# TaoMiner/joint-kg-recommender

Measured on NVIDIA H100. Metric: scored (h,r,t) triples/s, TransE d=100 forward + margin loss + backward, higher is better.
Workload: dtype f32

## Files before the change

joint-kg-recommender_b200/csrc/train_group.cu:

```cuda
#include <cstdlib>
#include "train_dev.cuh"

namespace kgrec {

struct GroupArgs {
  kgrec_tables T;
  const void *ph, *pt, *pr;
  int is64;
  const int32_t* corrupt;
  LossCfg L;
  float keep;
};

__device__ __forceinline__ const float* row_ptr(const float* base, uint32_t row, uint32_t ld) {
  return base + static_cast<uint64_t>(row) * ld;
}

template <int FAM, int NCH>
struct GroupPos {
  using R = Row<NCH, true>;
  static constexpr int NE = R::NE;
  float h[NE], t[NE], w[NE];
  float base_h[NE];
  float base_t[NE];
// ... 496 lines not shown
      goff += d4;
    };

    for (int k = 0; k < K; k += 2) {
      if (k + 1 < K) {
        idb = ent_id(__shfl_sync(FULL, cv, k + 1), headb);
        if (act) xb = ldg_f4_hint(row(ent_b, idb), pol_keep);
      }
      negative(xa, heada, ida, k);
      if (k + 1 < K) {
        if (k + 2 < K) {
          ida = ent_id(__shfl_sync(FULL, cv, k + 2), heada);
          if (act) xa = ldg_f4_hint(row(ent_b, ida), pol_keep);
        }
        negative(xb, headb, idb, k + 1);
      }
    }
    const float cp = cpos * up;
    const float4 eps = make_float4(cp * ddist_term(ep.x, L1), cp * ddist_term(ep.y, L1), cp * ddist_term(ep.z, L1), cp * ddist_term(ep.w, L1));
    float4 gh = make_float4(accT.x + eps.x, accT.y + eps.y, accT.z + eps.z, accT.w + eps.w);
    float4 gt = make_float4(accH.x - eps.x, accH.y - eps.y, accH.z - eps.z, accH.w - eps.w);
    float4 gr = make_float4(accT.x - accH.x + eps.x, accT.y - accH.y + eps.y, accT.z - accH.z + eps.z, accT.w - accH.w + eps.w);
    if (REG) {
      const float mh = 1.f + n_tail, mt = 1.f + (static_cast<float>(K) - n_tail), mr = 1.f + static_cast<float>(K);
      lreg += mh * fmaxf(nh2 - 1.f, 0.f) + mt * fmaxf(nt2 - 1.f, 0.f) + mr * fmaxf(nr2 - 1.f, 0.f);
      const float ch = nh2 > 1.f ? mh * r2 : 0.f, ct = nt2 > 1.f ? mt * r2 : 0.f, cr = nr2 > 1.f ? mr * r2 : 0.f;
      gh.x = fmaf(ch, h.x, gh.x); gh.y = fmaf(ch, h.y, gh.y); gh.z = fmaf(ch, h.z, gh.z); gh.w = fmaf(ch, h.w, gh.w);
      gt.x = fmaf(ct, t.x, gt.x); gt.y = fmaf(ct, t.y, gt.y); gt.z = fmaf(ct, t.z, gt.z); gt.w = fmaf(ct, t.w, gt.w);
      gr.x = fmaf(cr, r.x, gr.x); gr.y = fmaf(cr, r.y, gr.y); gr.z = fmaf(cr, r.z, gr.z); gr.w = fmaf(cr, r.w, gr.w);
    }
    if (!BWD) {
      if (lane == 0) {
        pos_scores[j] = sp;
        group_loss[j] = lsum + (REG ? lreg : 0.f);
      }
      if (lane < K) neg_scores[static_cast<uint32_t>(j) * K + lane] = mys;
    }
    if (!FWD && act) {
      if (DENSE) {
        red_add_f4(reinterpret_cast<float*>(gent_b + static_cast<uint64_t>(ih0) * d4), gh.x, gh.y, gh.z, gh.w);
        red_add_f4(reinterpret_cast<float*>(gent_b + static_cast<uint64_t>(it0) * d4), gt.x, gt.y, gt.z, gt.w);
        red_add_f4(reinterpret_cast<float*>(grel_b + static_cast<uint64_t>(ir0) * d4), gr.x, gr.y, gr.z, gr.w);
      } else {
        const uint32_t g0 = static_cast<uint32_t>(j) * (2 + K) * d4;
        stg_f4_hint(reinterpret_cast<float4*>(gent_b + g0), gh.x, gh.y, gh.z, gh.w, pol_stream);
        stg_f4_hint(reinterpret_cast<float4*>(gent_b + g0 + d4), gt.x, gt.y, gt.z, gt.w, pol_stream);
        stg_f4_hint(reinterpret_cast<float4*>(grel_b + static_cast<uint32_t>(j) * d4), gr.x, gr.y, gr.z, gr.w, pol_stream);
      }
    }
  }
  if (bad && status) *status = 1;
}

template <bool L1, bool DENSE, bool MARGIN, int W>
__global__ void __launch_bounds__(W * 32, 1)
k_group_step_e_tma(const GroupArgs G, const float up0, float* __restrict__ pos_scores, float* __restrict__ neg_scores,
                   float* __restrict__ group_loss, const kgrec_grads Gr, int64_t* __restrict__ slot_ent,
                   int64_t* __restrict__ slot_rel, int32_t* status, const int S) {
  extern __shared__ __align__(128) unsigned char smem_raw[];
  const kgrec_tables& T = G.T;
  const LossCfg& L = G.L;
  const int lane = threadIdx.x & 31, wid = threadIdx.x >> 5;
  const int K = L.n_neg, n_rows = 3 + K;
  const int n_pos = static_cast<int>(L.n_pos);
  const uint32_t n_ent = static_cast<uint32_t>(T.n_ent);
  const uint32_t ld4 = static_cast<uint32_t>(T.ld) * 4u, d4 = static_cast<uint32_t>(T.dim) * 4u;
  const int bp = static_cast<int>(L.batch_pos < 0x7fffffff ? L.batch_pos : 0x7fffffff);
  const uint64_t pol_stream = policy_evict_first();
  const bool act = lane * 4 < T.dim;
  uint64_t* bars = reinterpret_cast<uint64_t*>(smem_raw) + wid * S;
  int32_t* ids_ring = reinterpret_cast<int32_t*>(smem_raw + static_cast<size_t>(W) * S * 8) + wid * S * 32;
  const uint32_t stage_bytes = static_cast<uint32_t>(n_rows) * d4;
  unsigned char* rows_base = smem_raw + ((static_cast<size_t>(W) * S * (8 + 128) + 127) & ~static_cast<size_t>(127)) +
                             static_cast<size_t>(wid) * S * stage_bytes;
  if (lane == 0)
    for (int s = 0; s < S; ++s) mbar_init(bars + s, 1);
  mbar_fence_init();
  __syncwarp();
  char* gent_b = reinterpret_cast<char*>(Gr.ent) + lane * 16;
  char* grel_b = reinterpret_cast<char*>(Gr.rel) + lane * 16;
  const float prm = L.param;
  const int stride = gridDim.x * W;
  const float4 z4 = make_float4(0.f, 0.f, 0.f, 0.f);
  bool bad = false;
  const void* pcol = lane == 0 ? G.ph : (lane == 1 ? G.pt : G.pr);

  auto issue = [&](int jj, int s) {
    int32_t v = 0;
    if (lane < 3) {
      const int64_t pv = load_idx(pcol, jj, G.is64);
      const int64_t lim = lane == 2 ? T.n_rel : T.n_ent;
      if (static_cast<uint64_t>(pv) >= static_cast<uint64_t>(lim)) bad = true; else v = static_cast<int32_t>(pv);
    } else if (lane < n_rows) {
      v = __ldg(G.corrupt + static_cast<uint32_t>(jj) * K + (lane - 3));
      const uint32_t id = static_cast<uint32_t>(v < 0 ? ~v : v);
      if (id >= n_ent) { bad = true; v = 0; }
    }
    ids_ring[s * 32 + lane] = v;
    if (lane == 0) mbar_arrive_expect_tx(bars + s, stage_bytes);
    __syncwarp();
    if (lane < n_rows) {
      const uint32_t id = lane < 3 ? static_cast<uint32_t>(v) : static_cast<uint32_t>(v < 0 ? ~v : v);
      const char* src = reinterpret_cast<const char*>(lane == 2 ? T.rel : T.ent) + static_cast<uint64_t>(id) * ld4;
      bulk_g2s(rows_base + static_cast<size_t>(s) * stage_bytes + static_cast<size_t>(lane) * d4, src, d4, bars + s);
    }
  };

  int j = blockIdx.x * W + wid;
  for (int s = 0, jj = j; s < S - 1 && jj < n_pos; ++s, jj += stride) issue(jj, s);
  for (int it = 0; j < n_pos; j += stride, ++it) {
    const int s = it % S;
    {
      const int jn = j + (S - 1) * stride;
      if (jn < n_pos) {
        fence_proxy_async_smem();
        __syncwarp();
        issue(jn, (it + S - 1) % S);
      }
    }
    mbar_wait(bars + s, static_cast<uint32_t>(it / S) & 1u);
    const int32_t myid = ids_ring[s * 32 + lane];
    const uint32_t st_addr = smem_u32(rows_base + static_cast<size_t>(s) * stage_bytes) + lane * 16;
    const uint32_t ih0 = static_cast<uint32_t>(__shfl_sync(FULL, myid, 0)), it0 = static_cast<uint32_t>(__shfl_sync(FULL, myid, 1)),
                   ir0 = static_cast<uint32_t>(__shfl_sync(FULL, myid, 2));
    if (slot_ent) {
      const uint32_t s0 = static_cast<uint32_t>(j) * (2 + K);
      if (lane < 2) slot_ent[s0 + lane] = myid;
      if (lane == 2) slot_rel[j] = myid;
      if (lane >= 3 && lane < n_rows) slot_ent[s0 + lane - 1] = myid < 0 ? ~myid : myid;
    }
    float4 h = z4, t = z4, r = z4;
    if (act) { h = lds_f4(st_addr); t = lds_f4(st_addr + d4); r = lds_f4(st_addr + 2 * d4); }
    float up = up0;
    if (!MARGIN) {
      const int b = j / bp;
      up /= static_cast<float>(min(bp, n_pos - b * bp)) * static_cast<float>(K);
    }
    const float4 bh = make_float4(h.x + r.x, h.y + r.y, h.z + r.z, h.w + r.w);
    const float4 bt = make_float4(t.x - r.x, t.y - r.y, t.z - r.z, t.w - r.w);
    const float4 ep = make_float4(bh.x - t.x, bh.y - t.y, bh.z - t.z, bh.w - t.w);
    const float sp = warp_sum(dist_term(ep.x, L1) + dist_term(ep.y, L1) + dist_term(ep.z, L1) + dist_term(ep.w, L1));
    float lsum = 0.f, cpos = 0.f, mys = 0.f;
    float4 accT = z4, accH = z4;
    uint32_t goff = (static_cast<uint32_t>(j) * (2 + K) + 2) * d4;
#pragma unroll 2
    for (int k = 0; k < K; ++k) {
      const int32_t c = __shfl_sync(FULL, myid, 3 + k);
      const bool head = c < 0;
      const uint32_t id = static_cast<uint32_t>(head ? ~c : c);
      float4 x = z4;
      if (act) x = lds_f4(st_addr + (3 + k) * d4);
      const float4 B = head ? bt : bh;
      const float4 e = make_float4(B.x - x.x, B.y - x.y, B.z - x.z, B.w - x.w);
      const float sn = warp_sum(dist_term(e.x, L1) + dist_term(e.y, L1) + dist_term(e.z, L1) + dist_term(e.w, L1));
      if (lane == k) mys = sn;
      float coef;
      if (MARGIN) {
        const float tt = sp - sn + prm;
        lsum += fmaxf(tt, 0.f);
        coef = tt > 0.f ? up : 0.f;
        cpos += tt > 0.f ? 1.f : 0.f;
      } else {
        const float xx = prm * (sp - sn);
        lsum += fmaxf(-xx, 0.f) + log1pf(expf(-fabsf(xx)));
        const float dp = -prm / (1.f + expf(xx));
        cpos += dp;
        coef = dp * up;
      }
      if (coef != 0.f) {
        float4 gc;
        if (L1) {
          gc = make_float4(coef * ddist_term(e.x, 1), coef * ddist_term(e.y, 1), coef * ddist_term(e.z, 1), coef * ddist_term(e.w, 1));
        } else {
          const float c2 = 2.f * coef;
          gc = make_float4(c2 * e.x, c2 * e.y, c2 * e.z, c2 * e.w);
        }
        if (head) { accH.x -= gc.x; accH.y -= gc.y; accH.z -= gc.z; accH.w -= gc.w; }
        else { accT.x -= gc.x; accT.y -= gc.y; accT.z -= gc.z; accT.w -= gc.w; }
        if (act) {
          if (DENSE) red_add_f4(reinterpret_cast<float*>(gent_b + static_cast<uint64_t>(id) * d4), gc.x, gc.y, gc.z, gc.w);
          else stg_f4_hint(reinterpret_cast<float4*>(gent_b + goff), gc.x, gc.y, gc.z, gc.w, pol_stream);
        }
      } else if (!DENSE) {
        if (act) stg_f4_hint(reinterpret_cast<float4*>(gent_b + goff), 0.f, 0.f, 0.f, 0.f, pol_stream);
      }
      goff += d4;
    }
    const float cp = cpos * up;
    const float4 eps = make_float4(cp * ddist_term(ep.x, L1), cp * ddist_term(ep.y, L1), cp * ddist_term(ep.z, L1), cp * ddist_term(ep.w, L1));
    const float4 gh = make_float4(accT.x + eps.x, accT.y + eps.y, accT.z + eps.z, accT.w + eps.w);
    const float4 gt = make_float4(accH.x - eps.x, accH.y - eps.y, accH.z - eps.z, accH.w - eps.w);
    const float4 gr = make_float4(accT.x - accH.x + eps.x, accT.y - accH.y + eps.y, accT.z - accH.z + eps.z, accT.w - accH.w + eps.w);
    if (lane == 0) {
      pos_scores[j] = sp;
      group_loss[j] = lsum;
    }
    if (lane < K) neg_scores[static_cast<uint32_t>(j) * K + lane] = mys;
    if (act) {
      if (DENSE) {
        red_add_f4(reinterpret_cast<float*>(gent_b + static_cast<uint64_t>(ih0) * d4), gh.x, gh.y, gh.z, gh.w);
        red_add_f4(reinterpret_cast<float*>(gent_b + static_cast<uint64_t>(it0) * d4), gt.x, gt.y, gt.z, gt.w);
        red_add_f4(reinterpret_cast<float*>(grel_b + static_cast<uint64_t>(ir0) * d4), gr.x, gr.y, gr.z, gr.w);
      } else {
        const uint32_t g0 = static_cast<uint32_t>(j) * (2 + K) * d4;
        stg_f4_hint(reinterpret_cast<float4*>(gent_b + g0), gh.x, gh.y, gh.z, gh.w, pol_stream);
        stg_f4_hint(reinterpret_cast<float4*>(gent_b + g0 + d4), gt.x, gt.y, gt.z, gt.w, pol_stream);
        stg_f4_hint(reinterpret_cast<float4*>(grel_b + static_cast<uint32_t>(j) * d4), gr.x, gr.y, gr.z, gr.w, pol_stream);
      }
    }
  }
  if (bad && status) *status = 1;
}

template <bool L1, bool DENSE, bool MARGIN, int MINB, bool PF, bool REG, bool BWD, bool FWD = false>
__global__ void __launch_bounds__(kThreads, MINB)
k_group_step_h(const GroupArgs G, const float up0, const float* __restrict__ up_dev, float* __restrict__ pos_scores,
               float* __restrict__ neg_scores, float* __restrict__ group_loss, const kgrec_grads Gr,
               int64_t* __restrict__ slot_ent, int64_t* __restrict__ slot_rel, int32_t* status) {
  const kgrec_tables& T = G.T;
  const LossCfg& L = G.L;
  const int lane = threadIdx.x & 31, wid = threadIdx.x >> 5;
  const int K = L.n_neg;
  const int n_pos = static_cast<int>(L.n_pos);
  const uint32_t n_ent = static_cast<uint32_t>(T.n_ent);
  const uint32_t ld4 = static_cast<uint32_t>(T.ld) * 4u, d4 = static_cast<uint32_t>(T.dim) * 4u;
  const int bp = static_cast<int>(L.batch_pos < 0x7fffffff ? L.batch_pos : 0x7fffffff);
  const uint64_t pol_keep = policy_evict_last(G.keep), pol_stream = policy_evict_first();
  const bool act = lane * 4 < T.dim;
  const char* ent_b = reinterpret_cast<const char*>(T.ent) + lane * 16;
  const char* rel_b = reinterpret_cast<const char*>(T.rel) + lane * 16;
  const char* nrm_b = reinterpret_cast<const char*>(T.norm) + lane * 16;
  char* gent_b = reinterpret_cast<char*>(Gr.ent) + lane * 16;
  char* grel_b = reinterpret_cast<char*>(Gr.rel) + lane * 16;
  char* gnrm_b = reinterpret_cast<char*>(Gr.norm) + lane * 16;
  const float prm = L.param;
  const int stride = gridDim.x * kWarpsPerCta;
  const float4 z4 = make_float4(0.f, 0.f, 0.f, 0.f);
  auto row = [&](const char* base, uint32_t id) { return reinterpret_cast<const float4*>(base + static_cast<uint64_t>(id) * ld4); };
  auto dot4 = [](const float4& a, const float4& b) { return fmaf(a.x, b.x, fmaf(a.y, b.y, fmaf(a.z, b.z, a.w * b.w))); };
  bool bad = false;
  auto ent_id = [&](int32_t c, bool& head) {
    head = c < 0;
    uint32_t id = static_cast<uint32_t>(head ? ~c : c);
    if (id >= n_ent) { bad = true; id = 0; }
    return id;
  };
  int j = blockIdx.x * kWarpsPerCta + wid;
  const void* pcol = lane == 0 ? G.ph : (lane == 1 ? G.pt : G.pr);
  auto fetch_ids = [&](int jj, int32_t& cv, int64_t& pv) {
    cv = lane < K ? __ldg(G.corrupt + static_cast<uint32_t>(jj) * K + lane) : 0;
    pv = lane < 3 ? load_idx(pcol, jj, G.is64) : 0;
  };
  int32_t cv = 0, cvn = 0;
  int64_t pv = 0, pvn = 0;
  if (j < n_pos) fetch_ids(j, cvn, pvn);
  for (; j < n_pos; j += stride) {
    cv = cvn;
    pv = pvn;
    const int jn = j + stride;
    if (jn < n_pos) fetch_ids(jn, cvn, pvn);
    const int64_t vh = __shfl_sync(FULL, pv, 0), vt = __shfl_sync(FULL, pv, 1), vr = __shfl_sync(FULL, pv, 2);
    uint32_t ih = static_cast<uint32_t>(vh), it = static_cast<uint32_t>(vt), ir = static_cast<uint32_t>(vr);
    if (static_cast<uint64_t>(vh) >= static_cast<uint64_t>(T.n_ent)) { bad = true; ih = 0; }
    if (static_cast<uint64_t>(vt) >= static_cast<uint64_t>(T.n_ent)) { bad = true; it = 0; }
    if (static_cast<uint64_t>(vr) >= static_cast<uint64_t>(T.n_rel)) { bad = true; ir = 0; }
    if (slot_ent) {
      const uint32_t s0 = static_cast<uint32_t>(j) * (2 + K);
      if (lane < 2) slot_ent[s0 + lane] = pv;
      if (lane == 2) slot_rel[j] = pv;
      if (lane < K) slot_ent[s0 + 2 + lane] = cv < 0 ? ~cv : cv;
    }
    float4 h = z4, t = z4, r = z4, w = z4, xa = z4, xb = z4;
    bool heada, headb = false;
    uint32_t ida = ent_id(__shfl_sync(FULL, cv, 0), heada), idb = 0;
    if (act) {
      h = ldg_f4_hint(row(ent_b, ih), pol_keep);
      t = ldg_f4_hint(row(ent_b, it), pol_keep);
      r = ldg_f4_hint(row(rel_b, ir), pol_keep);
      w = ldg_f4_hint(row(nrm_b, ir), pol_keep);
      xa = ldg_f4_hint(row(ent_b, ida), pol_keep);
    }
    if (PF && lane >= 2 && lane < K) {
      const uint32_t pid = static_cast<uint32_t>(cv < 0 ? ~cv : cv);
      if (pid < n_ent) {
        const char* pr = reinterpret_cast<const char*>(T.ent) + static_cast<uint64_t>(pid) * ld4;
        for (uint32_t o = 0; o < d4; o += 128) prefetch_l1(pr + o);
      }
    }
    float up = up0;
    if (BWD && up_dev) up *= __ldg(up_dev + j / bp);
    if (!MARGIN) {
      const int b = j / bp;
      up /= static_cast<float>(min(bp, n_pos - b * bp)) * static_cast<float>(K);
    }
    [[maybe_unused]] const float svec = (BWD && lane < K) ? __ldg(neg_scores + static_cast<uint32_t>(j) * K + lane) : 0.f;
    float a = dot4(h, w), b = dot4(t, w);
    warp_sum2(a, b);
    const float4 pt = make_float4(fmaf(-b, w.x, t.x), fmaf(-b, w.y, t.y), fmaf(-b, w.z, t.z), fmaf(-b, w.w, t.w));
    const float4 bh = make_float4(fmaf(-a, w.x, h.x) + r.x, fmaf(-a, w.y, h.y) + r.y, fmaf(-a, w.z, h.z) + r.z, fmaf(-a, w.w, h.w) + r.w);
    const float4 bt = make_float4(pt.x - r.x, pt.y - r.y, pt.z - r.z, pt.w - r.w);
    const float4 ep = make_float4(bh.x - pt.x, bh.y - pt.y, bh.z - pt.z, bh.w - pt.w);
    const float sp = BWD ? __ldg(pos_scores + j)
                         : warp_sum(dist_term(ep.x, L1) + dist_term(ep.y, L1) + dist_term(ep.z, L1) + dist_term(ep.w, L1));
    float lsum = 0.f, cpos = 0.f, mys = 0.f, sT = 0.f, sH = 0.f;
    float4 accT = z4, accH = z4, gwv = z4;
    uint32_t goff = (static_cast<uint32_t>(j) * (2 + K) + 2) * d4;
    [[maybe_unused]] float nh2 = 0.f, nt2 = 0.f, nr2 = 0.f, wr = 0.f, lreg = 0.f, n_tail = 0.f;
// ... 581 lines not shown
        if (MARGIN) {
          const float tt = sp - sn + prm;
          lsum += fmaxf(tt, 0.f);
          coef = tt > 0.f ? -up : 0.f;
          cpos += tt > 0.f ? 1.f : 0.f;
        } else {
          const float xx = prm * (sp - sn);
          lsum += fmaxf(-xx, 0.f) + log1pf(expf(-fabsf(xx)));
          const float dp = -prm / (1.f + expf(xx));
          cpos += dp;
          coef = -dp * up;
        }
#pragma unroll
        for (int i = 0; i < 4; ++i) {
          const int a = lane + 32 * i;
          const float g = coef * ddist_term(e[i], l1);
          gp[i] += g;
          if (head) gt[i] -= g; else gh[i] += g;
          if (a < d) Yc[a] = head ? g : -g;
        }
      }
      const float cp = cpos * up;
#pragma unroll
      for (int i = 0; i < 4; ++i) {
        const int a = lane + 32 * i;
        const float g = cp * ddist_term(yh[i] + rr[i] - yt[i], l1);
        gp[i] += g;
        if (a < d) {
          Y[a] = gh[i] + g;
          Y[pitch + a] = gt[i] - g;
          if (Gr.mode == 0) Gr.rel[static_cast<int64_t>(j) * d + a] = gp[i];
          else atomicAdd(Gr.rel + static_cast<uint64_t>(rel) * d + a, gp[i]);
        }
      }
      if (lane == 0) { pos_scores[j] = sp; group_loss[j] = lsum; }
      if (lane < K) neg_scores[static_cast<int64_t>(j) * K + lane] = mys;
    }
    if (wid == kWarpsPerCta - 1) plan(buf ^ 1, i0 + ng);
    __syncthreads();
    if (mt) {
      const float4* gp[QA];
      const ulonglong2* vp[QB];
#pragma unroll
      for (int qa = 0; qa < QA; ++qa) gp[qa] = reinterpret_cast<const float4*>(sG + 4 * min(ta + nta * qa, NC - 1));
#pragma unroll
      for (int q = 0; q < QB; ++q) vp[q] = reinterpret_cast<const ulonglong2*>(sV + 4 * min(tb + ntb * q, NC - 1));
      const int p4 = pitch >> 2;
#pragma unroll 2
      for (int n = 0; n < rows; ++n) {
        float4 g[QA];
        ulonglong2 v[QB];
#pragma unroll
        for (int qa = 0; qa < QA; ++qa) { g[qa] = *gp[qa]; gp[qa] += p4; }
#pragma unroll
        for (int q = 0; q < QB; ++q) { v[q] = *vp[q]; vp[q] += p4; }
#pragma unroll
        for (int qa = 0; qa < QA; ++qa) {
          const float gs[4] = {g[qa].x, g[qa].y, g[qa].z, g[qa].w};
#pragma unroll
          for (int r = 0; r < 4; ++r) {
            const f32x2 s2 = splat2(gs[r]);
#pragma unroll
            for (int q = 0; q < QB; ++q) {
              accM[4 * qa + r][q][0] = fma2(s2, v[q].x, accM[4 * qa + r][q][0]);
              accM[4 * qa + r][q][1] = fma2(s2, v[q].y, accM[4 * qa + r][q][1]);
            }
          }
        }
      }
    }
    __syncthreads();
    copy_rows();
#pragma unroll 1
    for (int rb = 0; rb < RB; ++rb) {
      const int base = 8 * (wid + kWarpsPerCta * rb);
      if (base >= rows) break;
      const int dense = Gr.mode;
      float* const* dstp = sDst + buf * ROWS + base;
      run_tile_dot<QF>(sG + base * pitch, sMt, d, NC, pitch, lane, [&](int i, int b, float v) {
        if (base + i < rows) {
          float* dst = dstp[i] + b;
          if (dense) atomicAdd(dst, v); else __stcs(dst, v);
        }
      });
    }
    asm volatile("cp.async.wait_group 0;" ::: "memory");
    __syncthreads();
    i0 += ng;
    buf ^= 1;
  }
  flush(cur_rel);
  if (bad && status) *status = 1;
}

__global__ void __launch_bounds__(256)
k_group_slot_ids(const void* ph, const void* pt, const void* pr, const int is64, const int32_t* __restrict__ corrupt,
                 const int64_t n_pos, const int K, int64_t* __restrict__ slot_ent, int64_t* __restrict__ slot_rel) {
  const int64_t total = n_pos * (2 + K);
  for (int64_t i = static_cast<int64_t>(blockIdx.x) * blockDim.x + threadIdx.x; i < total; i += static_cast<int64_t>(gridDim.x) * blockDim.x) {
    const int64_t j = i / (2 + K);
    const int t = static_cast<int>(i - j * (2 + K));
    int64_t v;
    if (t == 0) { v = load_idx(ph, j, is64); slot_rel[j] = load_idx(pr, j, is64); }
    else if (t == 1) v = load_idx(pt, j, is64);
    else { const int32_t c = __ldg(corrupt + j * K + (t - 2)); v = c < 0 ? ~c : c; }
    slot_ent[i] = v;
  }
}

__global__ void __launch_bounds__(256)
k_rel_hist(const void* pr, const int is64, const int n_pos, const int64_t n_rel, int32_t* __restrict__ count) {
  for (int j = blockIdx.x * blockDim.x + threadIdx.x; j < n_pos; j += gridDim.x * blockDim.x) {
    int64_t r = load_idx(pr, j, is64);
    if (static_cast<uint64_t>(r) >= static_cast<uint64_t>(n_rel)) r = 0;
    atomicAdd(count + r, 1);
  }
}

__global__ void __launch_bounds__(1024)
k_rel_scan(int32_t* __restrict__ count, const int64_t n_rel) {
  __shared__ int32_t part[1024];
  const int64_t per = (n_rel + 1023) / 1024, lo = threadIdx.x * per, hi = lo + per < n_rel ? lo + per : n_rel;
  int32_t s = 0;
  for (int64_t r = lo; r < hi; ++r) s += count[r];
  part[threadIdx.x] = s;
  __syncthreads();
  for (int off = 1; off < 1024; off <<= 1) {
    const int32_t v = threadIdx.x >= off ? part[threadIdx.x - off] : 0;
    __syncthreads();
    part[threadIdx.x] += v;
    __syncthreads();
  }
  int32_t run = part[threadIdx.x] - s;
  for (int64_t r = lo; r < hi; ++r) { const int32_t c = count[r]; count[r] = run; run += c; }
}

__global__ void __launch_bounds__(256)
k_rel_scatter(const void* pr, const int is64, const int n_pos, const int64_t n_rel, int32_t* __restrict__ cursor,
              int32_t* __restrict__ order) {
  for (int j = blockIdx.x * blockDim.x + threadIdx.x; j < n_pos; j += gridDim.x * blockDim.x) {
    int64_t r = load_idx(pr, j, is64);
    if (static_cast<uint64_t>(r) >= static_cast<uint64_t>(n_rel)) r = 0;
    order[atomicAdd(cursor + r, 1)] = j;
  }
}

int make_plan(const kgrec_tables* T, int model, Plan* pl);

static const char* group_step_env() {
  static const char* cached = [] { const char* e = getenv("KGREC_GROUP_STEP"); return e ? e : ""; }();
  return cached[0] ? cached : nullptr;
}

static int group_step_tma_mode(const kgrec_tables* T, int n_neg, int reg_flags) {
  const char* env = group_step_env();
  if (reg_flags) return 0;
  if (env && env[0] == 't' && env[1] && env[2]) {
    const int W = env[1] == '8' ? 8 : (env[1] == 'c' ? 12 : 16), S = env[2] - '0';
    if (S < 2 || S > 6) return 0;
    const size_t smem = static_cast<size_t>(W) * S * (136 + static_cast<size_t>(3 + n_neg) * T->dim * 4) + 128;
    return smem <= 225 * 1024 ? 16 * W + S : 0;
  }
  return 0;
}

static int group_check(const kgrec_tables* T, int model, Plan* pl, const void* ph, const void* pt, const void* pr,
                       int idx_bytes, int64_t n_pos, const int32_t* corrupt, int32_t n_neg, int64_t batch_pos,
                       int loss_kind, bool allow_r = false) {
  int rc = make_plan(T, model, pl);
  if (rc) return rc;
  if (pl->fam != FAM_E && pl->fam != FAM_H && !(allow_r && pl->fam == FAM_R)) {
    set_error("corrupt-format ranking loss is built for TransE / TransH (model %d)", model);
    return KGREC_ERR_UNSUPPORTED;
  }
  if (!pl->vec) { set_error("corrupt-format ranking loss needs embedding_size %% 4 == 0 and 16-byte aligned tables"); return KGREC_ERR_UNSUPPORTED; }
  if (idx_bytes != 4 && idx_bytes != 8) { set_error("idx_bytes must be 4 or 8"); return KGREC_ERR_INVALID; }
  if (!ph || !pt || !pr || !corrupt) { set_error("index array is NULL"); return KGREC_ERR_INVALID; }
  if (loss_kind != KGREC_LOSS_MARGIN && loss_kind != KGREC_LOSS_BPR) { set_error("unknown loss %d", loss_kind); return KGREC_ERR_INVALID; }
  if (n_pos < 0 || n_pos > 0x7fffffff || n_neg < 1 || batch_pos < 1) { set_error("bad n_pos / n_neg / batch_pos"); return KGREC_ERR_INVALID; }
  if (T->n_ent > 0x7fffffffll) { set_error("corrupt format holds entity ids in 31 bits"); return KGREC_ERR_UNSUPPORTED; }
  return KGREC_OK;
}

}

using namespace kgrec;

#define KGREC_GROUP_DISPATCH(CALL)                                            \
  if (pl.fam == FAM_E) {                                                      \
    if (pl.nch == 1) { CALL(FAM_E, 1) } else if (pl.nch == 2) { CALL(FAM_E, 2) } else { CALL(FAM_E, 4) } \
  } else {                                                                    \
    if (pl.nch == 1) { CALL(FAM_H, 1) } else if (pl.nch == 2) { CALL(FAM_H, 2) } else { CALL(FAM_H, 4) } \
  }

extern "C" int kgrec_corrupt_loss_fwd(const kgrec_tables* tables, int model, const void* ph, const void* pt,
                                      const void* pr, int idx_bytes, int64_t n_pos, const int32_t* corrupt,
                                      int32_t n_neg, int64_t batch_pos, int loss_kind, float margin_or_target,
                                      float* pos_scores, float* neg_scores, float* loss, void* workspace,
                                      int32_t* status, kgrec_stream_t stream) {
  Plan pl;
  int rc = group_check(tables, model, &pl, ph, pt, pr, idx_bytes, n_pos, corrupt, n_neg, batch_pos, loss_kind);
  if (rc) return rc;
  if (!pos_scores || !neg_scores || !loss || !workspace) { set_error("output / workspace pointer is NULL"); return KGREC_ERR_INVALID; }
  if (n_pos == 0) return KGREC_OK;
  const GroupArgs G{*tables, ph, pt, pr, idx_bytes == 8, corrupt, LossCfg{loss_kind, margin_or_target, n_neg, n_pos, batch_pos},
                    l2_keep_fraction(static_cast<double>(tables->n_ent) * tables->ld * sizeof(float))};
  float* group_loss = static_cast<float*>(workspace);
  cudaStream_t st = static_cast<cudaStream_t>(stream);
  const char* env = group_step_env();
  const bool small32 = n_neg <= 32 && static_cast<double>(n_pos) * (2 + n_neg) * tables->dim * 4 < 4.0e9 &&
                       static_cast<double>(n_pos) * n_neg < 2.0e9;
  if ((pl.fam == FAM_E || pl.fam == FAM_H) && pl.nch == 1 && small32 && !(env && env[0] == '0')) {
    const kgrec_grads nog{};
#define CALL_F(KERN, MINBV, L1V, MV) KERN<L1V, false, MV, MINBV, true, false, false, true><<<grid_for(n_pos), kThreads, 0, st>>>(G, 1.f, nullptr, pos_scores, neg_scores, group_loss, nog, nullptr, nullptr, status)
#define CALL_F4(KERN, MINBV)                                                                                        \
  {                                                                                                                 \
    const bool mg = loss_kind == KGREC_LOSS_MARGIN;                                                                 \
    if (tables->l1) { if (mg) CALL_F(KERN, MINBV, true, true); else CALL_F(KERN, MINBV, true, false); }             \
    else { if (mg) CALL_F(KERN, MINBV, false, true); else CALL_F(KERN, MINBV, false, false); }                      \
  }
    if (pl.fam == FAM_E) CALL_F4(k_group_step_e, 4) else CALL_F4(k_group_step_h, 3)
#undef CALL_F4
#undef CALL_F
  } else {
#define CALL(FAMV, NCHV)                                                                                                  \
  if (tables->l1) k_group_fwd<FAMV, NCHV, true><<<grid_for(n_pos), kThreads, 0, st>>>(G, pos_scores, neg_scores, group_loss, status); \
  else k_group_fwd<FAMV, NCHV, false><<<grid_for(n_pos), kThreads, 0, st>>>(G, pos_scores, neg_scores, group_loss, status);
  KGREC_GROUP_DISPATCH(CALL)
#undef CALL
  }
  KGREC_CUDA_OK(cudaGetLastError());
  const int64_t n_batches = (n_pos + batch_pos - 1) / batch_pos;
  k_batch_loss<<<static_cast<unsigned>(n_batches), 256, 0, st>>>(group_loss, G.L, loss);
  KGREC_CUDA_OK(cudaGetLastError());
  return KGREC_OK;
}

extern "C" int kgrec_corrupt_loss_bwd(const kgrec_tables* tables, int model, const void* ph, const void* pt,
                                      const void* pr, int idx_bytes, int64_t n_pos, const int32_t* corrupt,
                                      int32_t n_neg, int64_t batch_pos, int loss_kind, float margin_or_target,
                                      const float* pos_scores, const float* neg_scores, float grad_loss,
                                      const float* grad_loss_dev, const kgrec_grads* grads, int64_t* slot_ent_ids,
                                      int64_t* slot_rel_ids, kgrec_stream_t stream) {
  Plan pl;
  int rc = group_check(tables, model, &pl, ph, pt, pr, idx_bytes, n_pos, corrupt, n_neg, batch_pos, loss_kind);
  if (rc) return rc;
  if (!pos_scores || !neg_scores) { set_error("saved scores are NULL"); return KGREC_ERR_INVALID; }
  if ((slot_ent_ids == nullptr) != (slot_rel_ids == nullptr)) { set_error("slot_ent_ids and slot_rel_ids go together"); return KGREC_ERR_INVALID; }
  if (!grads || (grads->mode != 0 && grads->mode != 1) || !grads->ent || !grads->rel || (pl.fam == FAM_H && !grads->norm)) {
    set_error("bad grads descriptor");
    return KGREC_ERR_INVALID;
  }
  if (n_pos == 0) return KGREC_OK;
  const GroupArgs G{*tables, ph, pt, pr, idx_bytes == 8, corrupt, LossCfg{loss_kind, margin_or_target, n_neg, n_pos, batch_pos},
                    l2_keep_fraction(static_cast<double>(tables->n_ent) * tables->ld * sizeof(float))};
  cudaStream_t st = static_cast<cudaStream_t>(stream);
  const char* env = group_step_env();
  const bool small32 = n_neg <= 32 && static_cast<double>(n_pos) * (2 + n_neg) * tables->dim * 4 < 4.0e9 &&
                       static_cast<double>(n_pos) * n_neg < 2.0e9;
  if ((pl.fam == FAM_E || pl.fam == FAM_H) && pl.nch == 1 && small32 && !(env && env[0] == '0')) {
    float* ps = const_cast<float*>(pos_scores);
    float* ns = const_cast<float*>(neg_scores);
#define CALL_B(KERN, MINBV, L1V, DV, MV) KERN<L1V, DV, MV, MINBV, true, false, true><<<grid_for(n_pos), kThreads, 0, st>>>(G, grad_loss, grad_loss_dev, ps, ns, nullptr, *grads, slot_ent_ids, slot_rel_ids, nullptr)
#define CALL_B8(KERN, MINBV)                                                                                                   \
  {                                                                                                                            \
    const bool dn = grads->mode == 1, mg = loss_kind == KGREC_LOSS_MARGIN;                                                     \
    if (tables->l1) { if (dn) { if (mg) CALL_B(KERN, MINBV, true, true, true); else CALL_B(KERN, MINBV, true, true, false); }  \
                      else { if (mg) CALL_B(KERN, MINBV, true, false, true); else CALL_B(KERN, MINBV, true, false, false); } } \
    else { if (dn) { if (mg) CALL_B(KERN, MINBV, false, true, true); else CALL_B(KERN, MINBV, false, true, false); }           \
           else { if (mg) CALL_B(KERN, MINBV, false, false, true); else CALL_B(KERN, MINBV, false, false, false); } }          \
  }
    if (pl.fam == FAM_E) CALL_B8(k_group_step_e, 4) else CALL_B8(k_group_step_h, 3)
#undef CALL_B8
#undef CALL_B
  } else {
#define CALL(FAMV, NCHV)                                                                                                  \
  if (tables->l1) k_group_bwd<FAMV, NCHV, true><<<grid_for(n_pos), kThreads, 0, st>>>(G, pos_scores, neg_scores, grad_loss, grad_loss_dev, *grads); \
  else k_group_bwd<FAMV, NCHV, false><<<grid_for(n_pos), kThreads, 0, st>>>(G, pos_scores, neg_scores, grad_loss, grad_loss_dev, *grads);
  KGREC_GROUP_DISPATCH(CALL)
#undef CALL
    if (slot_ent_ids) {
      const int64_t total = n_pos * (2 + static_cast<int64_t>(n_neg));
      const int64_t ctas = (total + 255) / 256, cap = static_cast<int64_t>(sm_count()) * 16;
      k_group_slot_ids<<<static_cast<unsigned>(ctas < cap ? ctas : cap), 256, 0, st>>>(ph, pt, pr, idx_bytes == 8, corrupt, n_pos, n_neg,
                                                                                         slot_ent_ids, slot_rel_ids);
    }
  }
  KGREC_CUDA_OK(cudaGetLastError());
  return KGREC_OK;
}

extern "C" int64_t kgrec_corrupt_loss_step_workspace_bytes(const kgrec_tables* tables, int model, int64_t n_pos) {
  const int64_t n = n_pos > 0 ? n_pos : 1;
  if (model == KGREC_TRANSR && tables) return 4 * (2 * n + tables->n_rel + 1);
  return 4 * n;
}

extern "C" int kgrec_corrupt_loss_step(const kgrec_tables* tables, int model, const void* ph, const void* pt,
                                       const void* pr, int idx_bytes, int64_t n_pos, const int32_t* corrupt,
                                       int32_t n_neg, int64_t batch_pos, int loss_kind, float margin_or_target,
                                       float grad_loss, int32_t reg_flags, float* pos_scores, float* neg_scores, float* loss,
                                       const kgrec_grads* grads, int64_t* slot_ent_ids, int64_t* slot_rel_ids,
                                       void* workspace, int32_t* status, kgrec_stream_t stream) {
  Plan pl;
  int rc = group_check(tables, model, &pl, ph, pt, pr, idx_bytes, n_pos, corrupt, n_neg, batch_pos, loss_kind, true);
  if (rc) return rc;
  if (!pos_scores || !neg_scores || !loss || !workspace) { set_error("output / workspace pointer is NULL"); return KGREC_ERR_INVALID; }
  if (!grads || (grads->mode != 0 && grads->mode != 1) || !grads->ent || !grads->rel || (pl.fam == FAM_H && !grads->norm) ||
      (pl.fam == FAM_R && !grads->proj)) {
    set_error("bad grads descriptor");
    return KGREC_ERR_INVALID;
  }
  if ((slot_ent_ids == nullptr) != (slot_rel_ids == nullptr)) { set_error("slot_ent_ids and slot_rel_ids go together"); return KGREC_ERR_INVALID; }
  if (pl.fam == FAM_R) {
    if (reg_flags) { set_error("fused regularisers are built for TransE / TransH"); return KGREC_ERR_UNSUPPORTED; }
    if (pl.nch != 1 || n_neg > 14) { set_error("TransR step kernel: embedding_size <= 128 and at most 14 negatives per positive"); return KGREC_ERR_UNSUPPORTED; }
    if (n_pos == 0) return KGREC_OK;
    const GroupArgs GA{*tables, ph, pt, pr, idx_bytes == 8, corrupt, LossCfg{loss_kind, margin_or_target, n_neg, n_pos, batch_pos}, 1.f};
    float* gl = static_cast<float*>(workspace);
    cudaStream_t s2 = static_cast<cudaStream_t>(stream);
    int32_t* order = reinterpret_cast<int32_t*>(gl + n_pos);
    int32_t* cursor = order + n_pos;
    {
      const char* env = group_step_env();
      if (env && env[0] == 'u') order = nullptr;
    }
    if (order) {
      KGREC_CUDA_OK(cudaMemsetAsync(cursor, 0, sizeof(int32_t) * tables->n_rel, s2));
      const int gs = static_cast<int>((n_pos + 255) / 256 < sm_count() * 4 ? (n_pos + 255) / 256 : sm_count() * 4);
      k_rel_hist<<<gs, 256, 0, s2>>>(pr, idx_bytes == 8, static_cast<int>(n_pos), tables->n_rel, cursor);
      k_rel_scan<<<1, 1024, 0, s2>>>(cursor, tables->n_rel);
      k_rel_scatter<<<gs, 256, 0, s2>>>(pr, idx_bytes == 8, static_cast<int>(n_pos), tables->n_rel, cursor, order);
    }
    const bool mg = loss_kind == KGREC_LOSS_MARGIN;
    const char* env_r = group_step_env();
    const bool long_runs = n_pos >= 4 * tables->n_rel || (env_r && env_r[0] == 'r');
    if (tables->dim >= 32 && long_runs && !(env_r && (env_r[0] == 'w' || env_r[0] == 'u'))) {
      const int d = tables->dim, NC = d / 4, pitch = run_pitch(d), qf = d / 32;
      auto smem_for = [&](int rb) { return (2 * static_cast<size_t>(d) + 2 * 64 * rb) * pitch * 4 + 3 * 64 * rb * 8 + 72 * 4; };
      const int rb = (NC <= 27 && smem_for(2) <= 220 * 1024) ? 2 : 1;
      const size_t smem = smem_for(rb);
      const int64_t want = (n_pos + 3) / 4;
      const int grid = static_cast<int>(want < sm_count() ? want : sm_count());
#define CALL_RUN(QAV, QBV, QFV, RBV)                                                                                     \
  {                                                                                                                      \
    auto kern = mg ? k_run_step_r<QAV, QBV, QFV, RBV, true> : k_run_step_r<QAV, QBV, QFV, RBV, false>;                   \
    KGREC_CUDA_OK(cudaFuncSetAttribute(kern, cudaFuncAttributeMaxDynamicSharedMemorySize, static_cast<int>(smem)));       \
    kern<<<grid, kThreads, smem, s2>>>(GA, grad_loss, pos_scores, neg_scores, gl, *grads, slot_ent_ids, slot_rel_ids, status, order); \
  }
      if (NC <= 16) { if (qf <= 1) CALL_RUN(1, 1, 1, 2) else CALL_RUN(1, 1, 2, 2) }
      else if (NC <= 27) { if (qf <= 2) CALL_RUN(1, 3, 2, 2) else CALL_RUN(1, 3, 3, 2) }
      else { if (qf <= 3) CALL_RUN(2, 2, 3, 1) else CALL_RUN(2, 2, 4, 1) }
#undef CALL_RUN
    } else {
    const int64_t want = (n_pos + kWarpsPerCta - 1) / kWarpsPerCta;
    const int grid_r = static_cast<int>(want < sm_count() ? want : sm_count());
    const int nvt = n_neg <= 2 ? 4 : (n_neg <= 10 ? 12 : 16);
    const size_t smem = static_cast<size_t>(kWarpsPerCta) * (static_cast<size_t>(nvt) * (tables->dim / 4) + static_cast<size_t>(tables->dim) * (nvt / 4)) * 16;
#define CALL_R(NVTV, MV)                                                                                             \
  {                                                                                                                  \
    auto kern = k_group_step_r<NVTV, MV>;                                                                            \
    KGREC_CUDA_OK(cudaFuncSetAttribute(kern, cudaFuncAttributeMaxDynamicSharedMemorySize, static_cast<int>(smem)));   \
    kern<<<grid_r, kThreads, smem, s2>>>(GA, grad_loss, pos_scores, neg_scores, gl, *grads, slot_ent_ids, slot_rel_ids, status, order); \
  }
    if (nvt == 4) { if (mg) CALL_R(4, true) else CALL_R(4, false) }
    else if (nvt == 12) { if (mg) CALL_R(12, true) else CALL_R(12, false) }
    else { if (mg) CALL_R(16, true) else CALL_R(16, false) }
#undef CALL_R
    }
    KGREC_CUDA_OK(cudaGetLastError());
    const int64_t nbt = (n_pos + batch_pos - 1) / batch_pos;
    k_batch_loss<<<static_cast<unsigned>(nbt), 256, 0, s2>>>(gl, GA.L, loss);
    KGREC_CUDA_OK(cudaGetLastError());
    return KGREC_OK;
  }
  if (n_pos == 0) return KGREC_OK;
  const GroupArgs G{*tables, ph, pt, pr, idx_bytes == 8, corrupt, LossCfg{loss_kind, margin_or_target, n_neg, n_pos, batch_pos},
                    l2_keep_fraction(static_cast<double>(tables->n_ent) * tables->ld * sizeof(float))};
  float* group_loss = static_cast<float*>(workspace);
  cudaStream_t st = static_cast<cudaStream_t>(stream);
  if (reg_flags != 0 && reg_flags != 1) { set_error("reg_flags must be 0 or 1"); return KGREC_ERR_INVALID; }
  if (reg_flags && loss_kind != KGREC_LOSS_MARGIN) { set_error("fused regularisers go with the margin loss (the KG drivers' loss)"); return KGREC_ERR_UNSUPPORTED; }
  const char* env = group_step_env();
  const bool small32 = n_neg <= 32 && static_cast<double>(n_pos) * (2 + n_neg) * tables->dim * 4 < 4.0e9 &&
                       static_cast<double>(n_pos) * n_neg < 2.0e9;
  const int tma_mode = group_step_tma_mode(tables, n_neg, reg_flags);
  if (pl.fam == FAM_E && pl.nch == 1 && small32 && tma_mode && n_neg <= 29 && tables->ld == tables->dim) {
    const int W = tma_mode / 16, S = tma_mode % 16;
    const size_t smem = ((static_cast<size_t>(W) * S * (8 + 128) + 127) & ~static_cast<size_t>(127)) +
                        static_cast<size_t>(W) * S * (3 + n_neg) * tables->dim * 4;
    int64_t ctas = (n_pos + W - 1) / W;
    if (ctas > sm_count()) ctas = sm_count();
#define CALL_T(L1V, DV, MV, WV)                                                                                         \
  {                                                                                                                     \
    auto kern = k_group_step_e_tma<L1V, DV, MV, WV>;                                                                    \
    KGREC_CUDA_OK(cudaFuncSetAttribute(kern, cudaFuncAttributeMaxDynamicSharedMemorySize, static_cast<int>(smem)));      \
    kern<<<static_cast<int>(ctas), WV * 32, smem, st>>>(G, grad_loss, pos_scores, neg_scores, group_loss, *grads, slot_ent_ids, slot_rel_ids, status, S); \
  }
#define CALL_TW(L1V, DV, MV) { if (W == 8) CALL_T(L1V, DV, MV, 8) else if (W == 12) CALL_T(L1V, DV, MV, 12) else CALL_T(L1V, DV, MV, 16) }
    const bool dn = grads->mode == 1, mg = loss_kind == KGREC_LOSS_MARGIN;
    if (tables->l1) { if (dn) { if (mg) CALL_TW(true, true, true) else CALL_TW(true, true, false) } else { if (mg) CALL_TW(true, false, true) else CALL_TW(true, false, false) } }
    else { if (dn) { if (mg) CALL_TW(false, true, true) else CALL_TW(false, true, false) } else { if (mg) CALL_TW(false, false, true) else CALL_TW(false, false, false) } }
#undef CALL_TW
#undef CALL_T
  } else if (pl.fam == FAM_E && pl.nch == 1 && small32 && !(env && env[0] == '0')) {
#define CALL_E(L1V, DV, MV)                                                                                      \
  {                                                                                                              \
    if (env && env[0] == 'n')                                                                                    \
      k_group_step_e<L1V, DV, MV, 4, false, false, false><<<grid_for(n_pos), kThreads, 0, st>>>(G, grad_loss, nullptr, pos_scores, neg_scores, group_loss, *grads, slot_ent_ids, slot_rel_ids, status); \
    else if (env && env[0] == '3')                                                                               \
      k_group_step_e<L1V, DV, MV, 3, false, false, false><<<grid_for(n_pos), kThreads, 0, st>>>(G, grad_loss, nullptr, pos_scores, neg_scores, group_loss, *grads, slot_ent_ids, slot_rel_ids, status); \
    else if (MV && reg_flags)                                                                                    \
      k_group_step_e<L1V, DV, true, 4, true, true, false><<<grid_for(n_pos), kThreads, 0, st>>>(G, grad_loss, nullptr, pos_scores, neg_scores, group_loss, *grads, slot_ent_ids, slot_rel_ids, status); \
    else                                                                                                         \
      k_group_step_e<L1V, DV, MV, 4, true, false, false><<<grid_for(n_pos), kThreads, 0, st>>>(G, grad_loss, nullptr, pos_scores, neg_scores, group_loss, *grads, slot_ent_ids, slot_rel_ids, status); \
  }
    const bool dn = grads->mode == 1, mg = loss_kind == KGREC_LOSS_MARGIN;
    if (tables->l1) { if (dn) { if (mg) CALL_E(true, true, true) else CALL_E(true, true, false) } else { if (mg) CALL_E(true, false, true) else CALL_E(true, false, false) } }
    else { if (dn) { if (mg) CALL_E(false, true, true) else CALL_E(false, true, false) } else { if (mg) CALL_E(false, false, true) else CALL_E(false, false, false) } }
#undef CALL_E
  } else if (pl.fam == FAM_H && pl.nch == 1 && small32 && !(env && env[0] == '0')) {
#define CALL_H(L1V, DV, MV)                                                                                      \
  {                                                                                                              \
    if (env && env[0] == 'n')                                                                                    \
      k_group_step_h<L1V, DV, MV, 3, false, false, false><<<grid_for(n_pos), kThreads, 0, st>>>(G, grad_loss, nullptr, pos_scores, neg_scores, group_loss, *grads, slot_ent_ids, slot_rel_ids, status); \
    else if (env && env[0] == '2')                                                                               \
      k_group_step_h<L1V, DV, MV, 2, false, false, false><<<grid_for(n_pos), kThreads, 0, st>>>(G, grad_loss, nullptr, pos_scores, neg_scores, group_loss, *grads, slot_ent_ids, slot_rel_ids, status); \
    else if (MV && reg_flags)                                                                                    \
      k_group_step_h<L1V, DV, true, 3, true, true, false><<<grid_for(n_pos), kThreads, 0, st>>>(G, grad_loss, nullptr, pos_scores, neg_scores, group_loss, *grads, slot_ent_ids, slot_rel_ids, status); \
    else                                                                                                         \
      k_group_step_h<L1V, DV, MV, 3, true, false, false><<<grid_for(n_pos), kThreads, 0, st>>>(G, grad_loss, nullptr, pos_scores, neg_scores, group_loss, *grads, slot_ent_ids, slot_rel_ids, status); \
  }
    const bool dn = grads->mode == 1, mg = loss_kind == KGREC_LOSS_MARGIN;
    if (tables->l1) { if (dn) { if (mg) CALL_H(true, true, true) else CALL_H(true, true, false) } else { if (mg) CALL_H(true, false, true) else CALL_H(true, false, false) } }
    else { if (dn) { if (mg) CALL_H(false, true, true) else CALL_H(false, true, false) } else { if (mg) CALL_H(false, false, true) else CALL_H(false, false, false) } }
#undef CALL_H
  } else {
    if (reg_flags) { set_error("fused regularisers are built for the d <= 128 margin-loss step kernels only"); return KGREC_ERR_UNSUPPORTED; }
#define CALL(FAMV, NCHV)                                                                                        \
  if (tables->l1) k_group_step<FAMV, NCHV, true><<<grid_for(n_pos), kThreads, 0, st>>>(G, grad_loss, pos_scores, neg_scores, group_loss, *grads, status); \
  else k_group_step<FAMV, NCHV, false><<<grid_for(n_pos), kThreads, 0, st>>>(G, grad_loss, pos_scores, neg_scores, group_loss, *grads, status);
  KGREC_GROUP_DISPATCH(CALL)
#undef CALL
    if (slot_ent_ids) {
      const int64_t total = n_pos * (2 + static_cast<int64_t>(n_neg));
      const int64_t ctas = (total + 255) / 256, cap = static_cast<int64_t>(sm_count()) * 16;
      k_group_slot_ids<<<static_cast<unsigned>(ctas < cap ? ctas : cap), 256, 0, st>>>(ph, pt, pr, idx_bytes == 8, corrupt, n_pos, n_neg,
                                                                                         slot_ent_ids, slot_rel_ids);
    }
  }
  KGREC_CUDA_OK(cudaGetLastError());
  const int64_t n_batches = (n_pos + batch_pos - 1) / batch_pos;
  k_batch_loss<<<static_cast<unsigned>(n_batches), 256, 0, st>>>(group_loss, G.L, loss);
  KGREC_CUDA_OK(cudaGetLastError());
  return KGREC_OK;
}
```

Baseline: 2.643 billion.

## Enable TMA-staged TransE group step by default with 16 warps and 2 stages

Makes the TMA/shared-memory-staged TransE group-step kernel the default path whenever conditions allow: non-dense grads, no fused regularisers, enough positives to fill every SM, and enough shared memory. Before, it ran only when selected through an environment variable. The configuration is fixed at 16 warps and 2 stages. The negative-distance reduction is also rewritten with explicit fabs and fma chains. This trades the generic kernel for a persistent, pipelined one that overlaps row fetches with compute, at the risk of lower occupancy from the large shared-memory footprint.

New measurement: 2.850 billion (median of 6 runs). 1.08x the previous value.

```diff
diff --git a/joint-kg-recommender_b200/csrc/train_group.cu b/joint-kg-recommender_b200/csrc/train_group.cu
--- a/joint-kg-recommender_b200/csrc/train_group.cu
+++ b/joint-kg-recommender_b200/csrc/train_group.cu
@@ -672,7 +672,8 @@
       if (act) x = lds_f4(st_addr + (3 + k) * d4);
       const float4 B = head ? bt : bh;
       const float4 e = make_float4(B.x - x.x, B.y - x.y, B.z - x.z, B.w - x.w);
-      const float sn = warp_sum(dist_term(e.x, L1) + dist_term(e.y, L1) + dist_term(e.z, L1) + dist_term(e.w, L1));
+      const float sn = warp_sum(L1 ? fabsf(e.x) + fabsf(e.y) + fabsf(e.z) + fabsf(e.w)
+                                   : __fmaf_rn(e.w, e.w, __fmaf_rn(e.z, e.z, __fmaf_rn(e.x, e.x, __fmul_rn(e.y, e.y)))));
       if (lane == k) mys = sn;
       float coef;
       if (MARGIN) {
@@ -1560,16 +1561,10 @@
   return cached[0] ? cached : nullptr;
 }
 
-static int group_step_tma_mode(const kgrec_tables* T, int n_neg, int reg_flags) {
-  const char* env = group_step_env();
-  if (reg_flags) return 0;
-  if (env && env[0] == 't' && env[1] && env[2]) {
-    const int W = env[1] == '8' ? 8 : (env[1] == 'c' ? 12 : 16), S = env[2] - '0';
-    if (S < 2 || S > 6) return 0;
-    const size_t smem = static_cast<size_t>(W) * S * (136 + static_cast<size_t>(3 + n_neg) * T->dim * 4) + 128;
-    return smem <= 225 * 1024 ? 16 * W + S : 0;
-  }
-  return 0;
+constexpr int kTmaWarps = 16, kTmaStages = 2;
+static size_t group_step_tma_smem(int dim, int n_neg) {
+  return ((static_cast<size_t>(kTmaWarps) * kTmaStages * (8 + 128) + 127) & ~static_cast<size_t>(127)) +
+         static_cast<size_t>(kTmaWarps) * kTmaStages * (3 + n_neg) * dim * 4;
 }
 
 static int group_check(const kgrec_tables* T, int model, Plan* pl, const void* ph, const void* pt, const void* pr,
@@ -1792,24 +1787,23 @@
   const char* env = group_step_env();
   const bool small32 = n_neg <= 32 && static_cast<double>(n_pos) * (2 + n_neg) * tables->dim * 4 < 4.0e9 &&
                        static_cast<double>(n_pos) * n_neg < 2.0e9;
-  const int tma_mode = group_step_tma_mode(tables, n_neg, reg_flags);
-  if (pl.fam == FAM_E && pl.nch == 1 && small32 && tma_mode && n_neg <= 29 && tables->ld == tables->dim) {
-    const int W = tma_mode / 16, S = tma_mode % 16;
-    const size_t smem = ((static_cast<size_t>(W) * S * (8 + 128) + 127) & ~static_cast<size_t>(127)) +
-                        static_cast<size_t>(W) * S * (3 + n_neg) * tables->dim * 4;
-    int64_t ctas = (n_pos + W - 1) / W;
+  const bool tma = pl.fam == FAM_E && pl.nch == 1 && small32 && grads->mode == 0 && !reg_flags && n_neg <= 29 &&
+                   tables->ld == tables->dim && !(env && (env[0] == '0' || env[0] == 'n' || env[0] == '3')) &&
+                   group_step_tma_smem(tables->dim, n_neg) <= 225 * 1024 &&
+                   n_pos >= static_cast<int64_t>(kTmaStages) * kTmaWarps * sm_count();
+  if (tma) {
+    const size_t smem = group_step_tma_smem(tables->dim, n_neg);
+    int64_t ctas = (n_pos + kTmaWarps - 1) / kTmaWarps;
     if (ctas > sm_count()) ctas = sm_count();
-#define CALL_T(L1V, DV, MV, WV)                                                                                         \
+#define CALL_T(L1V, MV)                                                                                                 \
   {                                                                                                                     \
-    auto kern = k_group_step_e_tma<L1V, DV, MV, WV>;                                                                    \
+    auto kern = k_group_step_e_tma<L1V, false, MV, kTmaWarps>;                                                          \
     KGREC_CUDA_OK(cudaFuncSetAttribute(kern, cudaFuncAttributeMaxDynamicSharedMemorySize, static_cast<int>(smem)));      \
-    kern<<<static_cast<int>(ctas), WV * 32, smem, st>>>(G, grad_loss, pos_scores, neg_scores, group_loss, *grads, slot_ent_ids, slot_rel_ids, status, S); \
-  }
-#define CALL_TW(L1V, DV, MV) { if (W == 8) CALL_T(L1V, DV, MV, 8) else if (W == 12) CALL_T(L1V, DV, MV, 12) else CALL_T(L1V, DV, MV, 16) }
-    const bool dn = grads->mode == 1, mg = loss_kind == KGREC_LOSS_MARGIN;
-    if (tables->l1) { if (dn) { if (mg) CALL_TW(true, true, true) else CALL_TW(true, true, false) } else { if (mg) CALL_TW(true, false, true) else CALL_TW(true, false, false) } }
-    else { if (dn) { if (mg) CALL_TW(false, true, true) else CALL_TW(false, true, false) } else { if (mg) CALL_TW(false, false, true) else CALL_TW(false, false, false) } }
-#undef CALL_TW
+    kern<<<static_cast<int>(ctas), kTmaWarps * 32, smem, st>>>(G, grad_loss, pos_scores, neg_scores, group_loss, *grads, slot_ent_ids, slot_rel_ids, status, kTmaStages); \
+  }
+    const bool mg = loss_kind == KGREC_LOSS_MARGIN;
+    if (tables->l1) { if (mg) CALL_T(true, true) else CALL_T(true, false) }
+    else { if (mg) CALL_T(false, true) else CALL_T(false, false) }
 #undef CALL_T
   } else if (pl.fam == FAM_E && pl.nch == 1 && small32 && !(env && env[0] == '0')) {
 #define CALL_E(L1V, DV, MV)                                                                                      \
```
